# rchikhi/rust-seq2kminmers

Measured on AMD Instinct MI355X. Metric: input bases/s (Gbp/s) for k-min-mer extraction, l=31 k=10 d=0.01, higher is better.
Workload: dtype u32

## Files before the change

### rust-seq2kminmers_amd/csrc/s2k_api.hip

```cpp
#include "../../include/s2k.h"
#include "s2k_dev.h"
#include "s2k_hostcopy.h"

#include <math.h>
#include <stdio.h>
#include <stdlib.h>
#include <string.h>
#include <string>
#include <algorithm>
#include <atomic>
#include <chrono>
#include <condition_variable>
#include <thread>
#include <memory>
#include <mutex>
#include <sys/mman.h>
#include <vector>

using namespace s2k;

static_assert(offsetof(Counts, path) == offsetof(s2k_counts, path), "Counts must start with s2k_counts");

namespace {

// ... 116 lines not shown
    bool pinned[9] = {};
    explicit HostOwner(std::shared_ptr<HostPool> hp) : pool(std::move(hp)) {}
    template <typename T> T *take(int slot, uint64_t n) {
        p[slot] = pool->get((size_t)n * sizeof(T), &cap[slot], &pinned[slot]);
        return (T *)p[slot];
    }
    ~HostOwner() {
        for (int i = 0; i < 9; i++) pool->put(p[i], cap[i], pinned[i]);
    }
};

struct DevBuf {
    void *p = nullptr;
    size_t bytes = 0;
    hipError_t ensure(size_t need) {
        if (need <= bytes) return hipSuccess;
        if (p) {
            hipError_t e = hipFree(p);
            p = nullptr;
            bytes = 0;
            if (e != hipSuccess) return e;
        }
        size_t want = need + need / 8 + 4096;
        hipError_t e = hipMalloc(&p, want);
        if (e != hipSuccess) return e;
        bytes = want;
        return hipSuccess;
    }
    void release() {
        if (p) (void)hipFree(p);
        p = nullptr;
        bytes = 0;
    }
};

constexpr uint32_t MAX_DESC_CHUNKS = 64;
constexpr size_t CTRL_XOR_OFF = (sizeof(Counts) + 255) & ~(size_t)255;
constexpr size_t CTRL_CURSORS_OFF = CTRL_XOR_OFF + XOR_SHARDS * sizeof(uint64_t);

struct Arena {
    char *base;
    size_t off, cap;
    template <class T> T *take(size_t n) {
        size_t o = (off + 255) & ~(size_t)255;
        off = o + n * sizeof(T);
        return base ? reinterpret_cast<T *>(base + o) : nullptr;
    }
};

struct Call {
    const uint8_t *d_bases = nullptr;
    const uint64_t *d_read_off = nullptr;
    uint64_t n_reads = 0, n_bases = 0;
    s2k_params params{};
    s2k_device_out out{};
    Sem sem{};
    uint32_t bound = 0;
    bool serial = false;
    bool desc_run = false;
    bool full_runs = false;
    bool legacy = false;
    uint64_t pool_cap = 0;
    uint64_t slab_cap = 0;
    bool valid = false;
};

}

struct s2k_ctx {
    int device = 0;
    hipStream_t stream = nullptr;
    bool user_stream = false;
    bool has_pipes = false;
    hipStream_t p = nullptr;
    hipEvent_t done_ev = nullptr;
    bool done_valid = false;
    hipEvent_t entry_ev = nullptr;
    DevBuf ws, in_bases, in_off, outbuf, realign;
    DevBuf in_bases2, in_off2, outbuf2;
    DevBuf count_tab;
    hipStream_t s_in = nullptr, s_out = nullptr;
    std::vector<hipEvent_t> chunk_ev;
    uint32_t rec_per_tile_hint = 0;
    s2k_ctx *chain_prev = nullptr;
    hipEvent_t tiles_done = nullptr;
    bool tiles_done_valid = false;
    uint32_t desc_chunks = 0;
    uint32_t lookback_giveups = 0;
    bool force_full_runs = false;
    bool trace = false;
    bool poison_ws = false;
    uint8_t poison_byte = 0;
    uint64_t host_batch = 1ull << 29;
    Counts *d_counts = nullptr;
    Counts *h_counts = nullptr;
    uint64_t *d_xor = nullptr;
    uint64_t *d_cursors = nullptr;
    std::vector<hipEvent_t> evs;
    size_t ev_used = 0;
    hipEvent_t *ev = nullptr;
    bool timing = false, timed = false;
    Call call;
    bool pending = false;
    s2k_status pending_status = S2K_OK;
    std::string err;
    s2k::HostStager stager;
    s2k::HostStager stager_out;
    std::shared_ptr<HostPool> host_pool = std::make_shared<HostPool>();
};

namespace {
std::mutex g_ctx_mu;
std::vector<s2k_ctx *> g_live_ctx;

struct PipePair {
    hipStream_t p = nullptr, k = nullptr;
    int refs = 0;
};
std::vector<PipePair> g_pipes;
}

namespace {
hipError_t ensure_pipes(s2k_ctx *ctx) {
    if (ctx->has_pipes) return hipSuccess;
    hipError_t e = hipSetDevice(ctx->device);
    if (e != hipSuccess) return e;
    std::lock_guard<std::mutex> lk(g_ctx_mu);
    if (g_pipes.size() <= (size_t)ctx->device) g_pipes.resize((size_t)ctx->device + 1);
    PipePair &pp = g_pipes[ctx->device];
    if (!pp.p) {
        hipStream_t p = nullptr, spacer = nullptr, k = nullptr;
        e = hipStreamCreateWithFlags(&p, hipStreamNonBlocking);
        if (e == hipSuccess) e = hipStreamCreateWithFlags(&spacer, hipStreamNonBlocking);
        if (e == hipSuccess) e = hipStreamCreateWithFlags(&k, hipStreamNonBlocking);
        if (spacer) (void)hipStreamDestroy(spacer);
        if (e != hipSuccess) {
            if (p) (void)hipStreamDestroy(p);
            if (k) (void)hipStreamDestroy(k);
            return e;
        }
        pp.p = p;
        pp.k = k;
    }
    pp.refs++;
    ctx->has_pipes = true;
    ctx->p = pp.p;
    if (!ctx->user_stream) ctx->stream = pp.k;
    return hipSuccess;
}

hipError_t mark_done(s2k_ctx *ctx) {
    hipError_t e = hipEventRecord(ctx->done_ev, ctx->stream);
    if (e == hipSuccess) ctx->done_valid = true;
    return e;
}
}

namespace s2k {
HostStager &ctx_stager(s2k_ctx *c) { return c->stager; }
hipStream_t ctx_stream(s2k_ctx *c) {
    (void)ensure_pipes(c);
    return c->stream;
}
hipError_t ctx_mark(s2k_ctx *c) { return mark_done(c); }
hipError_t ctx_sync(s2k_ctx *c) {
    hipError_t e = mark_done(c);
// ... 182 lines not shown
        rec.ovf_cursor = (unsigned long long *)pool_cursor;
        if (pass == 0) {
            S2K_TRY(ctx->ws.ensure(a.off + 256), "workspace allocation");
            a.base = (char *)ctx->ws.p;
        }
    }
    if (c.serial) {
        tile_cnt = mn_cnt;
        tile_goff = mn_off;
        tile_rec_off = mn_off;
    }

    const bool tm = ctx->timing;
    ctx->timed = tm;
    S2K_TRY(ensure_pipes(ctx), "stream create");
    hipStream_t const sp = ctx->p, sk = ctx->stream;
    while (ctx->chunk_ev.size() < (size_t)n_chunks) {
        hipEvent_t e;
        S2K_TRY(hipEventCreateWithFlags(&e, hipEventDisableTiming), "event create");
        ctx->chunk_ev.push_back(e);
    }
    if (!ctx->tiles_done) S2K_TRY(hipEventCreateWithFlags(&ctx->tiles_done, hipEventDisableTiming), "event create");
    if (tm) {
        if (ctx->evs.size() < (ctx->ev_used + 1) * 6) {
            for (int i = 0; i < 6; i++) {
                hipEvent_t e;
                S2K_TRY(hipEventCreate(&e), "event create");
                ctx->evs.push_back(e);
            }
        }
        ctx->ev = &ctx->evs[ctx->ev_used * 6];
        ctx->ev_used++;
    }
    if (ctx->user_stream) {
        S2K_TRY(hipEventRecord(ctx->entry_ev, sk), "event");
        S2K_TRY(hipStreamWaitEvent(sp, ctx->entry_ev, 0), "stream wait (entry)");
    } else if (ctx->done_valid && hipEventQuery(ctx->done_ev) != hipSuccess) {
        S2K_TRY(hipStreamWaitEvent(sp, ctx->done_ev, 0), "stream wait (previous call)");
    }
    if (tm) S2K_TRY(hipEventRecord(ctx->ev[0], sp), "event");
    S2K_TRY(hipMemsetAsync(ctx->d_counts, 0, CTRL_CURSORS_OFF + (size_t)CURSOR_WORDS * (use_desc ? n_chunks : 1) * sizeof(uint64_t), sp),
            "memset counters, xor shards, cursors");
    auto hand_over = [&]() -> s2k_status {
        S2K_TRY(hipEventRecord(ctx->tiles_done, sp), "event");
        ctx->tiles_done_valid = true;
        if (tm) S2K_TRY(hipEventRecord(ctx->ev[2], sp), "event");
        S2K_TRY(hipEventRecord(ctx->chunk_ev[0], sp), "event");
        S2K_TRY(hipStreamWaitEvent(sk, ctx->chunk_ev[0], 0), "stream wait");
        return S2K_OK;
    };
    if (c.serial) {
        S2K_TRY(launch_validate_read_off(c.d_read_off, n_reads, n_bases, &ctx->d_counts->bad_input, sp), "read table validation");
        if (tm) S2K_TRY(hipEventRecord(ctx->ev[1], sp), "event");
        S2K_TRY(launch_serial_count(c.d_bases, c.d_read_off, n_reads, n_bases, c.sem, mn_cnt, sp), "serial count kernel");
        S2K_TRY(launch_scan_u32(mn_cnt, n_reads, mn_off, scan_tmp, 0, sp), "scan");
        S2K_TRY(launch_serial_write(c.d_bases, c.d_read_off, n_reads, n_bases, c.sem, mn_off, rec, ctx->d_counts, sp), "serial write kernel");
        s2k_status hs = hand_over();
        if (hs != S2K_OK) return hs;
    } else {
        if (!use_desc) S2K_TRY(hipMemsetAsync(mn_cnt, 0, (n_reads + 1) * sizeof(uint32_t), sp), "memset mn_cnt");
        S2K_TRY(launch_read_table(c.d_read_off, n_reads, n_bases, n_tiles, &ctx->d_counts->bad_input, tile_read0,
                                  use_desc ? (unsigned long long *)d_agg : nullptr, agg_pack(0, 0, 0, 0, true, true), sp),
                "read table kernel");
        Sem sem = c.sem;
        sem.read_runs = nullptr;
        sem.tile_heads = nullptr;
        if (want_runs) {
            if (c.full_runs) {
                S2K_TRY(launch_read_run_counts(c.d_bases, c.d_read_off, n_reads, n_bases, run_blk, run_off, run_tmp, read_runs, nullptr, sp),
                        "run count kernels");
                sem.read_runs = read_runs;
            } else {
                S2K_TRY(hipMemsetAsync(tile_heads, 0, n_tiles * sizeof(uint32_t), sp), "memset tile head words");
                sem.tile_heads = tile_heads;
            }
        }
        const uint32_t tile_mode = tile_mode_of(sem);
        if (use_desc) {
            Desc dz{};
            dz.agg = d_agg;
            dz.meta = d_meta;
            dz.state = d_state;
            dz.k = c.sem.k;
            dz.spec_n = ctx->rec_per_tile_hint ? ctx->rec_per_tile_hint : 192u;
            dz.km_capacity = o.km_capacity;
            dz.mn_capacity = o.mn_capacity;
            dz.o_km_off = (unsigned long long *)o.km_off;
            dz.o_hash = (unsigned long long *)o.hash;
            dz.o_start = o.start;
            dz.o_end = o.end;
            dz.o_rev = o.rev;
            dz.o_mn_off = (unsigned long long *)mn_off;
            dz.o_mn_j = o.mn_j;
            dz.o_mn_jend = o.mn_jend;
            dz.o_mn_hash = o.mn_hash;
            dz.xor_shards = (unsigned long long *)ctx->d_xor;
            if (tm) S2K_TRY(hipEventRecord(ctx->ev[1], sp), "event");
            if (tm && n_chunks > 1) S2K_TRY(hipEventRecord(ctx->ev[3], sk), "event");
            for (uint32_t ch = 0; ch < n_chunks; ch++) {
                auto cut = [&](uint32_t i) -> uint64_t {
                    static const double tail = getenv("S2K_DESC_TAIL") ? atof(getenv("S2K_DESC_TAIL")) : 0.0;
                    if (i >= n_chunks) return n_tiles;
                    if (tail <= 0.0 || tail >= 1.0 || n_chunks < 2) return n_tiles * i / n_chunks;
                    return (uint64_t)((double)n_tiles * (1.0 - tail) * (double)i / (double)(n_chunks - 1));
                };
                const uint64_t T0 = cut(ch), T1 = cut(ch + 1);
                const bool last = ch + 1 == n_chunks;
                S2K_TRY(launch_tile_minimizers(c.d_bases, c.d_read_off, n_reads, n_bases, T1, tile_read0, sem, tile_mode, rec,
                                               pool_cursor + (size_t)CURSOR_WORDS * ch, nullptr, nullptr, nullptr, ctx->d_counts, &dz, T0, sp),
                        "tiled minimizer kernel");
                if (last) {
                    S2K_TRY(hipEventRecord(ctx->tiles_done, sp), "event");
                    ctx->tiles_done_valid = true;
                    if (tm) S2K_TRY(hipEventRecord(ctx->ev[2], sp), "event");
                }
                S2K_TRY(hipEventRecord(ctx->chunk_ev[ch], sp), "event");
                S2K_TRY(hipStreamWaitEvent(sk, ctx->chunk_ev[ch], 0), "stream wait");
                if (tm && n_chunks == 1) S2K_TRY(hipEventRecord(ctx->ev[3], sk), "event");
#ifdef S2K_DEBUG_KNOBS
                static const bool nokm = getenv("S2K_DEBUG_NOKM") != nullptr;
                if (nokm) continue;
#endif
                S2K_TRY(launch_desc_scan(T0, T1, dz, d_scan, ctx->d_counts, sk), "tile word scan");
                S2K_TRY(launch_desc_kminmers(T0, T1, n_tiles, n_reads, dz, rec, ctx->d_counts, sk, last && !(chained && c.sem.hpc)), "k-min-mer kernel");
            }
            if (tm) S2K_TRY(hipEventRecord(ctx->ev[4], sk), "event");
            S2K_TRY(launch_finalize(ctx->d_counts, ctx->d_xor, (const uint64_t *)&d_state[n_tiles].gmn, (const uint64_t *)&d_state[n_tiles].g,
                                    o.km_capacity, o.mn_capacity, sk),
                    "finalize kernel");
            S2K_TRY(hipMemcpyAsync(ctx->h_counts, ctx->d_counts, sizeof(Counts), hipMemcpyDeviceToHost, sk), "counts copy");
            if (tm) S2K_TRY(hipEventRecord(ctx->ev[5], sk), "event");
            S2K_TRY(mark_done(ctx), "event");
            ctx->pending = true;
            return S2K_OK;
        }
        if (tm) S2K_TRY(hipEventRecord(ctx->ev[1], sp), "event");
        S2K_TRY(launch_tile_minimizers(c.d_bases, c.d_read_off, n_reads, n_bases, n_tiles, tile_read0, sem, tile_mode, rec, pool_cursor,
                                       tile_rec_off, tile_cnt, mn_cnt, ctx->d_counts, nullptr, 0, sp),
                "tiled minimizer kernel");
        s2k_status hs = hand_over();
        if (hs != S2K_OK) return hs;
        S2K_TRY(launch_scan_u32(tile_cnt, n_tiles, tile_goff, scan_tmp, 0, sk), "scan");
        S2K_TRY(launch_scan_u32(mn_cnt, n_reads, mn_off, scan_tmp, 0, sk), "scan");
    }
    S2K_TRY(launch_scan_u32(mn_cnt, n_reads, o.km_off, scan_tmp, c.sem.k, sk), "scan");
    if (tm) S2K_TRY(hipEventRecord(ctx->ev[3], sk), "event");
    S2K_TRY(launch_kminmers(n_tiles, tile_rec_off, tile_cnt, tile_goff, rec, mn_off, o.km_off, c.sem.k, o.km_capacity, o.hash,
                            o.start, o.end, o.rev, o.mn_capacity, o.mn_capacity ? o.mn_j : nullptr, o.mn_jend, o.mn_hash,
                            ctx->d_xor, ctx->d_counts, sk),
            "k-min-mer kernel");
    if (tm) S2K_TRY(hipEventRecord(ctx->ev[4], sk), "event");
    S2K_TRY(launch_finalize(ctx->d_counts, ctx->d_xor, mn_off + n_reads, o.km_off + n_reads, o.km_capacity, o.mn_capacity, sk),
            "finalize kernel");
    S2K_TRY(hipMemcpyAsync(ctx->h_counts, ctx->d_counts, sizeof(Counts), hipMemcpyDeviceToHost, sk), "counts copy");
    if (tm) S2K_TRY(hipEventRecord(ctx->ev[5], sk), "event");
    S2K_TRY(mark_done(ctx), "event");
    ctx->pending = true;
    return S2K_OK;
}

s2k_status finish(s2k_ctx *ctx, s2k_counts *counts) {
    if (!ctx->pending) {
        if (counts && ctx->call.valid) memcpy(counts, ctx->h_counts, sizeof(s2k_counts));
        return ctx->pending_status;
    }
    for (int attempt = 0; attempt < 4; attempt++) {
        S2K_TRY(hipEventSynchronize(ctx->done_ev), "event synchronize");
        ctx->pending = false;
        Counts *h = ctx->h_counts;
        Call &c = ctx->call;
        if (h->bad_input) {
            ctx->pending_status = (h->bad_input & ~(uint32_t)BAD_LONG) ? S2K_ERR_INVALID_ARG : S2K_ERR_READ_TOO_LONG;
            ctx->err = (h->bad_input & BAD_FIRST)   ? "d_read_off[0] != 0"
                       : (h->bad_input & BAD_ORDER) ? "d_read_off is not non-decreasing"
                       : (h->bad_input & BAD_END)   ? "d_read_off[n_reads] != n_bases"
                                                    : "a read is longer than 2^32-2 bases";
            c.valid = false;
            return ctx->pending_status;
        }
        if (h->need_legacy && c.desc_run) {
            c.legacy = true;
            if (ctx->trace) fprintf(stderr, "[s2k] re-run: the descriptor path met a tile it does not handle -> legacy path\n");
            s2k_status st = enqueue(ctx);
            if (st != S2K_OK) return st;
            continue;
        }
        if (h->need_runs && !c.full_runs) {
            c.full_runs = true;
            if (++ctx->lookback_giveups >= 2) ctx->force_full_runs = true;
            if (ctx->trace) fprintf(stderr, "[s2k] re-run: a look-back for run heads gave up -> runs of every read counted first\n");
            s2k_status st = enqueue(ctx);
            if (st != S2K_OK) return st;
            continue;
        }
        if (h->pool_overflow) {
            c.pool_cap = h->pool_needed + h->pool_needed / 64 + (uint64_t)TILE_BASES + 4096;
            if (ctx->trace) fprintf(stderr, "[s2k] re-run: record pool too small -> %llu records\n", (unsigned long long)c.pool_cap);
            s2k_status st = enqueue(ctx);
            if (st != S2K_OK) return st;
            continue;
        }
        if (c.desc_run && c.n_bases >= 64u * (uint64_t)TILE_BASES) {
            const double avg = (double)h->n_minimizers / ((double)c.n_bases / (double)TILE_BASES);
            const double want = avg + 2.5 * sqrt(avg + 1.0) + 3.0;
            ctx->rec_per_tile_hint = want >= 192.0 ? 192u : (uint32_t)want;
        }
        h->n_reads = c.n_reads;
        h->n_bases = c.n_bases;
        h->hash_bound = c.bound;
        h->path = c.serial ? 1u : (c.desc_run ? 0u : 2u);
        if (c.sem.dbg_skip & 32)
        {
            fprintf(stderr, "[s2k dbg] last wave finished %.1f us after the first; shader clock under the tiled kernel %.0f MHz (waves alive %.3f ms on average)\n",
                    (double)(h->dbg_cycles[0][0] - ~h->dbg_cycles[0][1]) * 0.01,
                    h->dbg_cycles[1][1] ? 100.0 * (double)h->dbg_cycles[1][0] / (double)h->dbg_cycles[1][1] : 0.0,
                    (double)h->dbg_cycles[1][1] * 1e-5 / (256.0 * 12.0));
#ifdef S2K_DEBUG_KNOBS
            if (const char *path = getenv("S2K_DEBUG_WAVE_DUMP")) {
                if (FILE *f = fopen(path, "w")) {
                    for (int i = 0; i < 4096; i++)
                        if (h->dbg_wave[i][0]) fprintf(f, "%d %llu %u %u\n", i, (unsigned long long)(h->dbg_wave[i][0] - ~h->dbg_cycles[0][1]), (unsigned)(h->dbg_wave[i][1] >> 32), (unsigned)h->dbg_wave[i][1]);
                    fclose(f);
                }
            }
#endif
        }
        if (c.sem.dbg_skip & 8) {
            fprintf(stderr, "[s2k dbg] phase cycles (sum over waves):");
            for (int i = 0; i < 16; i++) {
                unsigned long long sum = 0;
                for (int sh = 0; sh < 64; sh++) sum += h->dbg_cycles[sh][i];
                fprintf(stderr, " %llu", sum);
            }
            fprintf(stderr, "\n");
        }
        if (counts) memcpy(counts, h, sizeof(s2k_counts));
        ctx->pending_status = (h->km_overflow || h->mn_overflow) ? S2K_ERR_CAPACITY : S2K_OK;
        if (ctx->pending_status != S2K_OK) ctx->err = "device output capacity too small; see counts";
        return ctx->pending_status;
    }
    return fail(ctx, S2K_ERR_DEVICE, "workspace retry did not converge");
}

}

extern "C" {

int s2k_abi_version(void) { return S2K_ABI_VERSION; }

double s2k_density_for_bound(uint32_t bound) {
    if (bound == 0xFFFFFFFFu) return 1.0;
    const double d = ((double)bound + 0.5) / 4294967295.0;
    return hash_bound(d) == bound ? d : ((double)bound + 0.25) / 4294967295.0;
}

int s2k_device_count(void) {
    int n = 0;
    if (hipGetDeviceCount(&n) != hipSuccess) return 0;
    return n;
}

const char *s2k_strerror(s2k_status st) {
    switch (st) {
    case S2K_OK: return "ok";
    case S2K_ERR_INVALID_ARG: return "invalid argument";
    case S2K_ERR_L_RANGE: return "minimizer length l out of range";
    case S2K_ERR_K_RANGE: return "k-min-mer order k out of range";
    case S2K_ERR_READ_TOO_LONG: return "a read is longer than 2^32-2 bases";
    case S2K_ERR_DEVICE: return "HIP runtime error";
    case S2K_ERR_NOMEM: return "out of memory";
    case S2K_ERR_CAPACITY: return "device output capacity too small";
    case S2K_ERR_NO_DEVICE: return "no GPU visible (this library has no CPU path)";
    case S2K_ERR_NON_ASCII: return "reserved (not returned since ABI 2: every byte value is accepted)";
    }
    return "unknown status";
}

const char *s2k_last_error(const s2k_ctx *ctx) { return ctx ? ctx->err.c_str() : "no context"; }

uint32_t s2k_hash_bound(double density) { return hash_bound(density); }

s2k_ctx *s2k_create(int device, s2k_status *status) {
    s2k_status dummy;
    if (!status) status = &dummy;
    int n = 0;
    if (hipGetDeviceCount(&n) != hipSuccess || n <= 0) {
        *status = S2K_ERR_NO_DEVICE;
        return nullptr;
    }
    if (device < 0 || device >= n) {
        *status = S2K_ERR_INVALID_ARG;
        return nullptr;
    }
    if (hipSetDevice(device) != hipSuccess) {
        *status = S2K_ERR_DEVICE;
        return nullptr;
    }
    s2k_ctx *ctx = new (std::nothrow) s2k_ctx();
    if (!ctx) {
        *status = S2K_ERR_NOMEM;
        return nullptr;
    }
    ctx->device = device;
    bool ok = hipEventCreateWithFlags(&ctx->done_ev, hipEventDisableTiming) == hipSuccess;
    ok = ok && hipEventCreateWithFlags(&ctx->entry_ev, hipEventDisableTiming) == hipSuccess;
    ok = ok && hipMalloc((void **)&ctx->d_counts, CTRL_CURSORS_OFF + (size_t)CURSOR_WORDS * MAX_DESC_CHUNKS * sizeof(uint64_t)) == hipSuccess;
    if (ok) {
        ctx->d_xor = reinterpret_cast<uint64_t *>(reinterpret_cast<char *>(ctx->d_counts) + CTRL_XOR_OFF);
        ctx->d_cursors = reinterpret_cast<uint64_t *>(reinterpret_cast<char *>(ctx->d_counts) + CTRL_CURSORS_OFF);
    }
    ok = ok && hipHostMalloc((void **)&ctx->h_counts, sizeof(Counts), hipHostMallocDefault) == hipSuccess;
    if (!ok) {
        *status = S2K_ERR_DEVICE;
        s2k_destroy(ctx);
        return nullptr;
    }
    memset(ctx->h_counts, 0, sizeof(Counts));
    if (const char *e = getenv("S2K_DESC_CHUNKS"))
        if (atoi(e) >= 1 && atoi(e) <= 64) ctx->desc_chunks = (uint32_t)atoi(e);
    if (const char *e = getenv("S2K_TRACE")) ctx->trace = atoi(e) != 0;
    if (const char *e = getenv("S2K_POISON_WS"))
        if (*e && atoi(e) >= 0 && atoi(e) <= 255) ctx->poison_ws = true, ctx->poison_byte = (uint8_t)atoi(e);
    if (const char *e = getenv("S2K_FULL_RUNS")) ctx->force_full_runs = atoi(e) != 0;
    {
        std::lock_guard<std::mutex> lk(g_ctx_mu);
        g_live_ctx.push_back(ctx);
    }
    *status = S2K_OK;
    return ctx;
}

void s2k_destroy(s2k_ctx *ctx) {
    if (!ctx) return;
    {
        std::lock_guard<std::mutex> lk(g_ctx_mu);
        for (size_t i = 0; i < g_live_ctx.size();) {
            if (g_live_ctx[i] == ctx) {
                g_live_ctx[i] = g_live_ctx.back();
                g_live_ctx.pop_back();
                continue;
            }
            if (g_live_ctx[i]->chain_prev == ctx) g_live_ctx[i]->chain_prev = nullptr;
            i++;
        }
    }
    (void)hipSetDevice(ctx->device);
    if (ctx->tiles_done_valid) (void)hipEventSynchronize(ctx->tiles_done);
    if (ctx->has_pipes) (void)s2k::ctx_sync(ctx);
    ctx->ws.release();
    ctx->in_bases.release();
    ctx->realign.release();
    ctx->in_off.release();
    ctx->outbuf.release();
    ctx->in_bases2.release();
    ctx->in_off2.release();
    ctx->outbuf2.release();
    ctx->count_tab.release();
    if (ctx->tiles_done) (void)hipEventDestroy(ctx->tiles_done);
    for (hipEvent_t e : ctx->chunk_ev) (void)hipEventDestroy(e);
    if (ctx->s_in) (void)hipStreamDestroy(ctx->s_in);
    if (ctx->s_out) (void)hipStreamDestroy(ctx->s_out);
    if (ctx->d_counts) (void)hipFree(ctx->d_counts);
    if (ctx->h_counts) (void)hipHostFree(ctx->h_counts);
    for (hipEvent_t e : ctx->evs) (void)hipEventDestroy(e);
    if (ctx->done_ev) (void)hipEventDestroy(ctx->done_ev);
    if (ctx->entry_ev) (void)hipEventDestroy(ctx->entry_ev);
    if (ctx->has_pipes) {
        std::lock_guard<std::mutex> lk(g_ctx_mu);
        PipePair &pp = g_pipes[ctx->device];
        if (--pp.refs == 0) {
            (void)hipStreamDestroy(pp.p);
            (void)hipStreamDestroy(pp.k);
            pp = PipePair();
        }
    }
    delete ctx;
}

s2k_status s2k_set_stream(s2k_ctx *ctx, void *hip_stream) {
    if (!ctx) return S2K_ERR_INVALID_ARG;
    if (ctx->pending) {
        s2k_status st = finish(ctx, nullptr);
        (void)st;
    }
    S2K_TRY(hipSetDevice(ctx->device), "set device");
    if (ctx->has_pipes) S2K_TRY(s2k::ctx_sync(ctx), "event synchronize");
    ctx->stream = (hipStream_t)hip_stream;
    ctx->user_stream = true;
    ctx->done_valid = false;
    return S2K_OK;
}

s2k_status s2k_chain_after(s2k_ctx *ctx, s2k_ctx *prev) {
    if (!ctx || prev == ctx) return S2K_ERR_INVALID_ARG;
    std::lock_guard<std::mutex> lk(g_ctx_mu);
    if (prev) {
        bool live = false;
        for (s2k_ctx *c : g_live_ctx) live = live || c == prev;
        if (!live || prev->device != ctx->device) return S2K_ERR_INVALID_ARG;
    }
    ctx->chain_prev = prev;
    return S2K_OK;
}

s2k_status s2k_enable_timing(s2k_ctx *ctx, int on) {
    if (!ctx) return S2K_ERR_INVALID_ARG;
// ... 557 lines not shown
```

### rust-seq2kminmers_amd/csrc/s2k_desc.hip

```cpp
#include "s2k_dev.h"
#include <cstdlib>
#include <type_traits>

namespace s2k {
namespace {

constexpr unsigned long long M48 = (1ull << 48) - 1ull;

struct PairState {
    uint64_t G, Gmn;
    uint32_t p;
};
__device__ inline PairState applied(PairState s, const AggF &a, uint32_t K1) {
    s.G += agg_windows(a, s.p, K1);
    s.Gmn += a.N;
    s.p = agg_p(a, s.p, K1);
    return s;
}
__device__ inline void st_agg(unsigned long long *w, const AggF &a) {
    w[0] = a.m_f;
    w[1] = a.C;
    w[2] = a.N;
    w[3] = (unsigned long long)a.q | ((unsigned long long)(a.dep ? 1 : 0) << 8) | ((unsigned long long)(a.pass ? 1 : 0) << 9);
}
// ... 27 lines not shown
        b.pass = (f & 512u) != 0;
        if (lane >= o) a = agg_then(b, a, K1);
    }
    return a;
}
__device__ inline bool scan_off(const Counts *counts) { return counts->need_legacy || counts->need_runs || counts->bad_input || counts->pool_overflow; }

template <bool PACKED>
__global__ __launch_bounds__(256) void desc_scan_reduce(const unsigned long long *__restrict__ in, uint64_t n, uint32_t K1,
                                                        unsigned long long *__restrict__ out, const Counts *__restrict__ counts) {
    const int lane = threadIdx.x & 63;
    const uint64_t c = (uint64_t)blockIdx.x * 4 + (threadIdx.x >> 6), i = c * 64 + lane;
    if (c * 64 >= n || scan_off(counts)) return;
    const AggF a = wave_scan_agg(i < n ? ld_level<PACKED>(in, i) : agg_identity(), lane, K1);
    if (lane == 63) st_agg(out + 4 * c, a);
}
__global__ __launch_bounds__(64) void desc_scan_top(const unsigned long long *__restrict__ in, uint64_t n, uint32_t K1,
                                                    unsigned long long *__restrict__ states, const TileState *__restrict__ init,
                                                    const Counts *__restrict__ counts) {
    const int lane = threadIdx.x;
    if (scan_off(counts)) return;
    PairState s{0, 0, 0};
    if (init) {
        s.G = init->g & M48;
        s.p = (uint32_t)(init->g >> 48) & 63u;
        s.Gmn = init->gmn;
    }
    for (uint64_t b0 = 0; b0 < n; b0 += 64) {
        const uint64_t i = b0 + lane;
        const AggF inc = wave_scan_agg(i < n ? ld_agg(in + 4 * i) : agg_identity(), lane, K1);
        AggF exc;
        exc.m_f = shfl_up64(inc.m_f, 1);
        exc.C = shfl_up64(inc.C, 1);
        exc.N = shfl_up64(inc.N, 1);
        const uint32_t f = (uint32_t)__shfl_up((int)(inc.q | (inc.dep ? 256u : 0u) | (inc.pass ? 512u : 0u)), 1);
        exc.q = f & 63u;
        exc.dep = (f & 256u) != 0;
        exc.pass = (f & 512u) != 0;
        if (lane == 0) exc = agg_identity();
        const PairState mine = applied(s, exc, K1);
        if (i < n) {
            states[3 * i] = mine.G;
            states[3 * i + 1] = mine.Gmn;
            states[3 * i + 2] = mine.p;
        }
        const PairState after = applied(s, inc, K1);
        s.G = ((uint64_t)(uint32_t)__shfl((int)(uint32_t)(after.G >> 32), 63) << 32) | (uint32_t)__shfl((int)(uint32_t)after.G, 63);
        s.Gmn = ((uint64_t)(uint32_t)__shfl((int)(uint32_t)(after.Gmn >> 32), 63) << 32) | (uint32_t)__shfl((int)(uint32_t)after.Gmn, 63);
        s.p = (uint32_t)__shfl((int)after.p, 63);
    }
}
template <bool PACKED>
__global__ __launch_bounds__(256) void desc_scan_expand(const unsigned long long *__restrict__ in, uint64_t n, uint32_t K1,
                                                        const unsigned long long *__restrict__ chunk_states, unsigned long long *__restrict__ out_states,
                                                        TileState *__restrict__ out_tiles, const Counts *__restrict__ counts) {
    const int lane = threadIdx.x & 63;
    const uint64_t c = (uint64_t)blockIdx.x * 4 + (threadIdx.x >> 6), i = c * 64 + lane;
    if (c * 64 >= n || scan_off(counts)) return;
    const PairState s0{chunk_states[3 * c], chunk_states[3 * c + 1], (uint32_t)chunk_states[3 * c + 2]};
    const AggF inc = wave_scan_agg(i < n ? ld_level<PACKED>(in, i) : agg_identity(), lane, K1);
    AggF exc;
    exc.m_f = shfl_up64(inc.m_f, 1);
    exc.C = shfl_up64(inc.C, 1);
    exc.N = shfl_up64(inc.N, 1);
    const uint32_t f = (uint32_t)__shfl_up((int)(inc.q | (inc.dep ? 256u : 0u) | (inc.pass ? 512u : 0u)), 1);
    exc.q = f & 63u;
    exc.dep = (f & 256u) != 0;
    exc.pass = (f & 512u) != 0;
    if (lane == 0) exc = agg_identity();
    const PairState mine = applied(s0, exc, K1);
    if (i < n) {
        if constexpr (PACKED) {
            out_tiles[i].g = ((unsigned long long)mine.p << 48) | mine.G;
            out_tiles[i].gmn = mine.Gmn;
            if (i + 1 == n) {
                const PairState tot = applied(s0, inc, K1);
                out_tiles[n].g = ((unsigned long long)tot.p << 48) | tot.G;
                out_tiles[n].gmn = tot.Gmn;
            }
        } else {
            out_states[3 * i] = mine.G;
            out_states[3 * i + 1] = mine.Gmn;
            out_states[3 * i + 2] = mine.p;
        }
    }
}

constexpr int DK_WAVES = 4;
constexpr int DK_KMAX = 32;

__device__ inline uint32_t dk_incl_scan(uint32_t v) {
    uint32_t t;
    t = (uint32_t)__builtin_amdgcn_update_dpp(0, (int)v, 0x111, 0xf, 0xf, false);
    uint32_t a = v + t;
    t = (uint32_t)__builtin_amdgcn_update_dpp(0, (int)v, 0x112, 0xf, 0xf, false);
    a += t;
    t = (uint32_t)__builtin_amdgcn_update_dpp(0, (int)v, 0x113, 0xf, 0xf, false);
    a += t;
    t = (uint32_t)__builtin_amdgcn_update_dpp(0, (int)a, 0x114, 0xf, 0xe, false);
    a += t;
    t = (uint32_t)__builtin_amdgcn_update_dpp(0, (int)a, 0x118, 0xf, 0xc, false);
    a += t;
    t = (uint32_t)__builtin_amdgcn_update_dpp(0, (int)a, 0x142, 0xa, 0xf, false);
    a += t;
    t = (uint32_t)__builtin_amdgcn_update_dpp(0, (int)a, 0x143, 0xc, 0xf, false);
    a += t;
    return a;
}
__device__ inline uint32_t dk_incl_xor(uint32_t v) {
    uint32_t t;
    t = (uint32_t)__builtin_amdgcn_update_dpp(0, (int)v, 0x111, 0xf, 0xf, false);
    uint32_t a = v ^ t;
    t = (uint32_t)__builtin_amdgcn_update_dpp(0, (int)v, 0x112, 0xf, 0xf, false);
    a ^= t;
    t = (uint32_t)__builtin_amdgcn_update_dpp(0, (int)v, 0x113, 0xf, 0xf, false);
    a ^= t;
    t = (uint32_t)__builtin_amdgcn_update_dpp(0, (int)a, 0x114, 0xf, 0xe, false);
    a ^= t;
    t = (uint32_t)__builtin_amdgcn_update_dpp(0, (int)a, 0x118, 0xf, 0xc, false);
    a ^= t;
    t = (uint32_t)__builtin_amdgcn_update_dpp(0, (int)a, 0x142, 0xa, 0xf, false);
    a ^= t;
    t = (uint32_t)__builtin_amdgcn_update_dpp(0, (int)a, 0x143, 0xc, 0xf, false);
    a ^= t;
    return a;
}
__device__ inline uint32_t dk_lane(uint32_t v, int src) { return (uint32_t)__builtin_amdgcn_readlane((int)v, src); }

constexpr int DK_STAGE_RECS = 192, DK_STAGE_BYTES = DK_STAGE_RECS * 20;
template <int KT, bool FULL, bool COAL = false>
__global__ __launch_bounds__(64 * DK_WAVES, 8) void desc_kminmer_kernel(uint64_t tile_begin, uint64_t tile_end, uint64_t n_tiles, uint64_t n_reads, Desc dz,
                                                                        Records rec, Counts *counts) {
    __shared__ unsigned long long s_ring[DK_WAVES][((KT > 0 && FULL) ? 32 : 64) + DK_KMAX];
    __shared__ uint4 s_seg[DK_WAVES][META_SEGS];
    __shared__ uint32_t s_jcar[DK_WAVES][DK_KMAX];
    const int lane = threadIdx.x & 63, w = __builtin_amdgcn_readfirstlane((int)(threadIdx.x >> 6));
    uint32_t *const s_cum_w = reinterpret_cast<uint32_t *>(&s_ring[w][DK_KMAX]);
    const uint64_t t = tile_begin + (uint64_t)blockIdx.x * DK_WAVES + w;
    if (t >= tile_end) return;
    const uint32_t off_flags = counts->need_legacy | counts->need_runs | counts->bad_input | counts->pool_overflow;
    const unsigned long long agw = t >= (uint64_t)lane ? dz.agg[t - lane] : 0ull;
    const TileState st = dz.state[t];
    const TileMeta *m = &dz.meta[t];
    const uint64_t base = m->rec_base, rs0 = m->rs0, t0 = t * (uint64_t)TILE_BASES;
    const uint32_t r0 = m->r0, nb = m->nb, nrd = m->nrd;
    const uint32_t segstart_raw = lane < META_SEGS ? m->segstart[lane] : 0u, rs16 = lane < META_SEGS ? m->rs16[lane] : 0u;
    const uint64_t slab = t * rec.slab_cap;
    uint32_t nh32 = rec.hash[slab + lane], npos = rec.j[slab + lane];
    constexpr bool KFIX = KT > 0;
    constexpr bool SERIAL = KFIX && FULL;
    uint32_t sp_h0 = 0, sp_h1 = 0, sp_h2 = 0, sp_p0 = 0, sp_p1 = 0, sp_p2 = 0;
    if constexpr (SERIAL) {
        if (3u * (uint32_t)lane < dz.spec_n) {
            const uint32_t *ph = rec.hash + slab + 3u * (uint32_t)lane, *pp = rec.j + slab + 3u * (uint32_t)lane;
            sp_h0 = ph[0], sp_h1 = ph[1], sp_h2 = ph[2];
            sp_p0 = pp[0], sp_p1 = pp[1], sp_p2 = pp[2];
        }
    }
    if (off_flags) return;
    const uint32_t k = KFIX ? (uint32_t)KT : dz.k, K1 = k - 1;
    const unsigned long long ag0 = ((unsigned long long)dk_lane((uint32_t)(agw >> 32), 0) << 32) | dk_lane((uint32_t)agw, 0);
    const AggF ag = agg_unpack(ag0);
    const uint32_t N = (uint32_t)ag.N;
    const uint64_t G = st.g & M48, Gmn = st.gmn;
    const uint32_t p_in = ag.dep ? (uint32_t)(st.g >> 48) & 63u : 0u;
    if (base != slab && (uint32_t)lane < N) {
// ... 329 lines not shown
#pragma unroll
            for (int mm = 0; mm < KT; mm++) {
                al[mm] = rot_lo(xl[mm], xh[mm], KT - 1 - mm);
                ah[mm] = rot_hi(xl[mm], xh[mm], KT - 1 - mm);
                bl[mm] = rot_lo(xl[mm], xh[mm], mm);
                bh[mm] = rot_hi(xl[mm], xh[mm], mm);
            }
            fl = al[0], fh = ah[0], rl = bl[0], rh = bh[0];
#pragma unroll
            for (int mm = 1; mm + 1 < KT; mm += 2) {
                fl = xor3(fl, al[mm], al[mm + 1]);
                fh = xor3(fh, ah[mm], ah[mm + 1]);
                rl = xor3(rl, bl[mm], bl[mm + 1]);
                rh = xor3(rh, bh[mm], bh[mm + 1]);
            }
            if constexpr (KT % 2 == 0) {
                fl ^= al[KT - 1];
                fh ^= ah[KT - 1];
                rl ^= bl[KT - 1];
                rh ^= bh[KT - 1];
            }
            rvv = ((uint64_t)rh << 32) | rl;
        } else {
            for (uint32_t mm = 0; mm < k; mm++) {
                const uint64_t xw = s_ring[w][lane + mm];
                const uint32_t xl = (uint32_t)xw, xh = (uint32_t)(xw >> 32);
                const uint32_t nfh = __builtin_amdgcn_alignbit(fh, fl, 31), nfl = __builtin_amdgcn_alignbit(fl, fh, 31);
                const uint32_t nrl = __builtin_amdgcn_alignbit(rh, rl, 1), nrh = __builtin_amdgcn_alignbit(rl, rh, 1);
                fl = nfl ^ xl;
                fh = nfh ^ xh;
                rl = nrl ^ xl;
                rh = nrh ^ xh;
            }
            rvv = rotl64(((uint64_t)rh << 32) | rl, K1);
        }
        const uint64_t f = ((uint64_t)fh << 32) | fl;
        const int src = ((lane - (int)K1) & 63) << 2;
        const uint32_t jsame = (uint32_t)__builtin_amdgcn_ds_bpermute(src, (int)j), jbefore = (uint32_t)__builtin_amdgcn_ds_bpermute(src, (int)jprev);
        const uint32_t jstart = (uint32_t)lane >= K1 ? jsame : jbefore;
        const uint64_t hmin = f < rvv ? f : rvv;
        if (win) {
            const uint32_t ot = i + sg.y;
            xacc ^= hmin;
            if (tile_fits) {
                t_hash[ot] = hmin;
                t_start[ot] = jstart;
                t_end[ot] = jend;
                t_rev[ot] = (uint8_t)(rvv < f);
            } else {
                const uint64_t o = G + (uint64_t)ot;
                if (o < dz.km_capacity) {
                    if (dz.o_hash) dz.o_hash[o] = hmin;
                    if (dz.o_start) dz.o_start[o] = jstart;
                    if (dz.o_end) dz.o_end[o] = jend;
                    if (dz.o_rev) dz.o_rev[o] = (uint8_t)(rvv < f);
                }
            }
        }
        if (!FULL && dz.mn_capacity && act) {
            const uint64_t g = Gmn + i;
            if (g < dz.mn_capacity) {
                dz.o_mn_j[g] = j;
                dz.o_mn_jend[g] = jend;
                dz.o_mn_hash[g] = h32;
            }
        }
        wave_sync();
        if ((uint32_t)lane >= 64u - K1) s_ring[w][lane - (64u - K1)] = xm;
        jprev = j;
    }
    }
    const uint32_t xl_all = dk_incl_xor((uint32_t)xacc), xh_all = dk_incl_xor((uint32_t)(xacc >> 32));
    if (lane == 63 && (xl_all | xh_all))
        atomicXor((unsigned long long *)&dz.xor_shards[t & (XOR_SHARDS - 1)], ((unsigned long long)xh_all << 32) | xl_all);
}

}

size_t desc_scan_tmp_words(uint64_t n_tiles) {
    const uint64_t n1 = (n_tiles + 63) / 64, n2 = (n1 + 63) / 64;
    return 7 * n1 + 7 * n2 + 16;
}

hipError_t launch_desc_scan(uint64_t tile_begin, uint64_t tile_end, Desc dz, unsigned long long *scan_tmp, const Counts *counts, hipStream_t st) {
    if (tile_end <= tile_begin) return hipSuccess;
    const uint64_t n = tile_end - tile_begin;
    const uint64_t n1 = (n + 63) / 64, n2 = (n1 + 63) / 64;
    unsigned long long *w1 = scan_tmp, *s1 = w1 + 4 * n1, *w2 = s1 + 3 * n1, *s2 = w2 + 4 * n2;
    const uint32_t K1 = dz.k - 1;
    const unsigned long long *agg = dz.agg + tile_begin;
    TileState *state = dz.state + tile_begin;
    hipLaunchKernelGGL(desc_scan_reduce<true>, dim3((unsigned)((n1 + 3) / 4)), dim3(256), 0, st, agg, n, K1, w1, counts);
    hipLaunchKernelGGL(desc_scan_reduce<false>, dim3((unsigned)((n2 + 3) / 4)), dim3(256), 0, st, w1, n1, K1, w2, counts);
    hipLaunchKernelGGL(desc_scan_top, dim3(1), dim3(64), 0, st, w2, n2, K1, s2, tile_begin ? (const TileState *)state : (const TileState *)nullptr, counts);
    hipLaunchKernelGGL(desc_scan_expand<false>, dim3((unsigned)((n2 + 3) / 4)), dim3(256), 0, st, w1, n1, K1, s2, s1, (TileState *)nullptr, counts);
    hipLaunchKernelGGL(desc_scan_expand<true>, dim3((unsigned)((n1 + 3) / 4)), dim3(256), 0, st, agg, n, K1, s1, (unsigned long long *)nullptr, state,
                       counts);
    return hipGetLastError();
}

hipError_t launch_desc_kminmers(uint64_t tile_begin, uint64_t tile_end, uint64_t n_tiles, uint64_t n_reads, Desc dz, Records rec, Counts *counts,
                                hipStream_t st, bool alone) {
    if (tile_end <= tile_begin) return hipSuccess;
    if (dz.k == 0 || dz.k > (uint32_t)DK_KMAX || rec.slab_cap < 64) return hipErrorInvalidValue;
    const dim3 g((unsigned)((tile_end - tile_begin + DK_WAVES - 1) / DK_WAVES)), b(64 * DK_WAVES);
    unsigned pad = 0;
#ifdef S2K_DEBUG_KNOBS
    if (const char *e = getenv("S2K_DEBUG_KM_LDS")) pad = (unsigned)atoi(e);
#endif
    const bool full = dz.o_hash && dz.o_start && dz.o_end && dz.o_rev && dz.mn_capacity == 0;
    static const bool no_coal = getenv("S2K_KM_NO_COAL") != nullptr;
    const bool coal = alone && full && !no_coal && (dz.k == 10 || dz.k == 5);
#define S2K_KM_GO(KT, F, C) \
    hipLaunchKernelGGL((desc_kminmer_kernel<KT, F, C>), g, b, (C) ? (unsigned)(DK_WAVES * DK_STAGE_BYTES) : pad, st, tile_begin, tile_end, n_tiles, n_reads, dz, rec, counts)
    switch (dz.k) {
    case 10: if (coal) S2K_KM_GO(10, true, true); else if (full) S2K_KM_GO(10, true, false); else S2K_KM_GO(10, false, false); break;
    case 5: if (coal) S2K_KM_GO(5, true, true); else if (full) S2K_KM_GO(5, true, false); else S2K_KM_GO(5, false, false); break;
    default: if (full) S2K_KM_GO(0, true, false); else S2K_KM_GO(0, false, false); break;
    }
#undef S2K_KM_GO
    return hipGetLastError();
}

}
```

### rust-seq2kminmers_amd/csrc/s2k_dev.h

```cpp
#pragma once
#include <hip/hip_runtime.h>
#include <stdint.h>

namespace s2k {

constexpr uint32_t SEED_A = 0x95c60474u, SEED_C = 0x62a02b4cu, SEED_G = 0x82572324u, SEED_T = 0x4be24456u;

__host__ __device__ inline uint32_t seed_h_scalar(uint32_t c) {
    return c == 'A' ? SEED_A : c == 'C' ? SEED_C : c == 'G' ? SEED_G : c == 'T' ? SEED_T : c == 'N' ? 0u : 1u;
}
__host__ __device__ inline uint32_t seed_rc_scalar(uint32_t c) {
    return c == 'A' ? SEED_T : c == 'C' ? SEED_G : c == 'G' ? SEED_C : c == 'T' ? SEED_A : c == 'N' ? 0u : 1u;
}
__host__ __device__ inline uint32_t seed_h_simd(uint32_t c) {
    uint32_t n = c & 15u;
    return n == 1 ? SEED_A : n == 3 ? SEED_C : n == 7 ? SEED_G : n == 4 ? SEED_T : 0u;
}
__host__ __device__ inline uint32_t seed_rc_simd(uint32_t c) {
    uint32_t n = c & 15u;
    return n == 1 ? SEED_T : n == 3 ? SEED_G : n == 7 ? SEED_C : n == 4 ? SEED_A : 0u;
}

#if defined(__HIP_DEVICE_COMPILE__)
__device__ __forceinline__ uint32_t xor3(uint32_t a, uint32_t b, uint32_t c) {
// ... 127 lines not shown
constexpr int META_SEGS = 32;
struct TileMeta {
    unsigned long long rec_base;
    unsigned long long rs0;
    uint32_t r0;
    uint16_t nb, nrd;
    uint16_t segstart[META_SEGS];
    uint16_t rs16[META_SEGS];
};
struct TileState {
    unsigned long long g;
    unsigned long long gmn;
};
constexpr uint32_t REC_SPAN_MAX = (1u << 18) - 1u;
struct Desc {
    unsigned long long *agg;
    TileMeta *meta;
    TileState *state;
    uint32_t k;
    uint32_t spec_n;
    unsigned long long km_capacity, mn_capacity;
    unsigned long long *o_km_off, *o_hash;
    uint32_t *o_start, *o_end;
    uint8_t *o_rev;
    unsigned long long *o_mn_off;
    uint32_t *o_mn_j, *o_mn_jend, *o_mn_hash;
    unsigned long long *xor_shards;
};

#define S2K_HIP_CHECK(expr)                                                      \
    do {                                                                         \
        hipError_t _e = (expr);                                                  \
        if (_e != hipSuccess) return _e;                                         \
    } while (0)

hipError_t launch_scan_u32(const uint32_t *in, uint64_t n, uint64_t *out , uint64_t *block_tmp,
                           uint32_t sub_k , hipStream_t st);
size_t scan_tmp_bytes(uint64_t n);

__host__ __device__ inline bool is_rle_char(uint32_t c) {
    const uint32_t d = (c & 0xDFu) - 'A';
    return d < 20u && ((0x82045u >> d) & 1u) != 0u;
}
__host__ __device__ inline bool run_head(uint32_t cur, uint32_t prev, bool rle) { return cur != prev || (rle && !is_rle_char(cur)); }

hipError_t launch_read_run_counts(const uint8_t *bases, const uint64_t *read_off, uint64_t n_reads, uint64_t n_bases,
                                  uint32_t *blk_cnt, uint64_t *blk_off, uint64_t *scan_tmp, uint32_t *runs, uint64_t *read_c0,
                                  hipStream_t st, bool rle = false);
hipError_t launch_hpc_segments(const uint8_t *bases, const uint64_t *read_off, uint64_t n_reads, uint64_t n_bases,
                               const uint64_t *hpc_off, const uint64_t *blk_off, const uint64_t *read_c0, uint32_t *seg_index, uint8_t *o_hpc,
                               uint32_t *o_pos, uint64_t capacity, hipStream_t st, bool rle = false);
size_t hpc_single_pass_words(uint64_t n_bases);
hipError_t launch_hpc_single_pass(const uint8_t *bases, const uint64_t *read_off, uint64_t n_reads, uint64_t n_bases, uint32_t *ws, uint64_t *o_hpc_off,
                                  uint8_t *o_hpc, uint32_t *o_pos, uint64_t capacity, uint32_t **fail_word, hipStream_t st, bool rle = false);
size_t hpc_segment_index_words(uint64_t n_bases);

hipError_t launch_validate_read_off(const uint64_t *read_off, uint64_t n_reads, uint64_t n_bases, uint32_t *bad, hipStream_t st);
hipError_t launch_read_table(const uint64_t *read_off, uint64_t n_reads, uint64_t n_bases, uint64_t n_tiles, uint32_t *bad, uint32_t *tile_read0,
                             unsigned long long *tile_words, unsigned long long word0, hipStream_t st);

hipError_t launch_synth(uint64_t seed, uint64_t first_base, uint64_t n, uint8_t *d, hipStream_t st);
hipError_t launch_fill_u64(unsigned long long *d, uint64_t n, unsigned long long v, hipStream_t st);
uint64_t synth_hifi_len(uint64_t seed, uint64_t r);
hipError_t launch_synth_hifi(uint64_t seed, uint64_t r0, uint64_t n_reads, const uint64_t *read_off, uint8_t *d, hipStream_t st);

hipError_t launch_serial_count(const uint8_t *bases, const uint64_t *read_off, uint64_t n_reads, uint64_t n_bases, Sem sem,
                               uint32_t *mn_cnt, hipStream_t st);
hipError_t launch_serial_write(const uint8_t *bases, const uint64_t *read_off, uint64_t n_reads, uint64_t n_bases, Sem sem,
                               const uint64_t *mn_off, Records rec, Counts *counts, hipStream_t st);

hipError_t launch_kminmers(uint64_t n_tiles, const uint64_t *tile_rec_off, const uint32_t *tile_cnt,
                           const uint64_t *tile_goff, Records rec, const uint64_t *mn_off, const uint64_t *km_off,
                           uint32_t k, uint64_t km_capacity, uint64_t *o_hash, uint32_t *o_start, uint32_t *o_end,
                           uint8_t *o_rev, uint64_t mn_capacity, uint32_t *o_mn_j, uint32_t *o_mn_jend,
                           uint32_t *o_mn_hash, uint64_t *xor_shards, const Counts *counts, hipStream_t st);
hipError_t launch_finalize(Counts *counts, const uint64_t *xor_shards, const uint64_t *mn_total, const uint64_t *km_total,
                           uint64_t km_capacity, uint64_t mn_capacity, hipStream_t st);

hipError_t launch_tile_minimizers(const uint8_t *bases, const uint64_t *read_off, uint64_t n_reads, uint64_t n_bases,
                                  uint64_t n_tiles, const uint32_t *tile_read0, Sem sem, uint32_t mode, Records rec,
                                  uint64_t *pool_cursor, uint64_t *tile_rec_off, uint32_t *tile_cnt, uint32_t *mn_cnt,
                                  Counts *counts, const Desc *desc, uint64_t tile_begin, hipStream_t st);
hipError_t launch_desc_scan(uint64_t tile_begin, uint64_t tile_end, Desc dz, unsigned long long *scan_tmp ,
                            const Counts *counts, hipStream_t st);
size_t desc_scan_tmp_words(uint64_t n_tiles);
hipError_t launch_desc_kminmers(uint64_t tile_begin, uint64_t tile_end, uint64_t n_tiles, uint64_t n_reads, Desc dz, Records rec, Counts *counts,
                                hipStream_t st, bool alone);

hipError_t launch_hpc_count(const uint8_t *bases, const uint64_t *read_off, uint64_t n_reads, uint32_t *run_cnt, hipStream_t st,
                            bool rle = false);
hipError_t launch_hpc_write(const uint8_t *bases, const uint64_t *read_off, uint64_t n_reads, const uint64_t *hpc_off,
                            uint8_t *o_hpc, uint32_t *o_pos, uint64_t capacity, hipStream_t st, bool rle = false);

enum { FX_TOT_RECORDS = 0, FX_TOT_BASES, FX_TOT_ERR, FX_TOT_BLANK, FX_TOT_LASTLINE, FX_TOT_NEWLINES, FX_N_TOTALS };
size_t fx_ws_bytes(uint64_t n);
bool fx_malformed(const uint64_t *h_totals, uint64_t n, int fastq);
hipError_t fx_parse_count(const uint8_t *d_raw, uint64_t n, int fastq, void *ws, uint64_t *d_totals, hipStream_t st);
hipError_t fx_parse_write(const uint8_t *d_raw, uint64_t n, int fastq, void *ws, uint64_t *d_totals, uint8_t *d_bases,
                          uint64_t bases_cap, uint64_t *d_read_off, uint64_t off_cap, hipStream_t st);

}
```

Baseline: 1842.

## Replace five-launch tile-word scan with two-launch reduce/expand scan

```diff
diff --git a/rust-seq2kminmers_amd/csrc/s2k_api.hip b/rust-seq2kminmers_amd/csrc/s2k_api.hip
--- a/rust-seq2kminmers_amd/csrc/s2k_api.hip
+++ b/rust-seq2kminmers_amd/csrc/s2k_api.hip
@@ -222,6 +222,12 @@
     hipStream_t s_in = nullptr, s_out = nullptr;
     std::vector<hipEvent_t> chunk_ev;
     uint32_t rec_per_tile_hint = 0;
+    struct {
+        int32_t mode = -1;
+        uint32_t l = 0, k = 0;
+        double density = 0.0;
+    } hint_key;
+    bool scan_five = false;
     s2k_ctx *chain_prev = nullptr;
     hipEvent_t tiles_done = nullptr;
     bool tiles_done_valid = false;
@@ -570,6 +576,8 @@
             dz.meta = d_meta;
             dz.state = d_state;
             dz.k = c.sem.k;
+            if (ctx->hint_key.mode != c.params.mode || ctx->hint_key.l != c.params.l || ctx->hint_key.k != c.params.k || ctx->hint_key.density != c.params.density)
+                ctx->rec_per_tile_hint = 0;
             dz.spec_n = ctx->rec_per_tile_hint ? ctx->rec_per_tile_hint : 192u;
             dz.km_capacity = o.km_capacity;
             dz.mn_capacity = o.mn_capacity;
@@ -609,7 +617,7 @@
                 static const bool nokm = getenv("S2K_DEBUG_NOKM") != nullptr;
                 if (nokm) continue;
 #endif
-                S2K_TRY(launch_desc_scan(T0, T1, dz, d_scan, ctx->d_counts, sk), "tile word scan");
+                S2K_TRY(launch_desc_scan(T0, T1, dz, d_scan, ctx->d_counts, sk, ctx->scan_five), "tile word scan");
                 S2K_TRY(launch_desc_kminmers(T0, T1, n_tiles, n_reads, dz, rec, ctx->d_counts, sk, last && !(chained && c.sem.hpc)), "k-min-mer kernel");
             }
             if (tm) S2K_TRY(hipEventRecord(ctx->ev[4], sk), "event");
@@ -692,6 +700,7 @@
             const double avg = (double)h->n_minimizers / ((double)c.n_bases / (double)TILE_BASES);
             const double want = avg + 2.5 * sqrt(avg + 1.0) + 3.0;
             ctx->rec_per_tile_hint = want >= 192.0 ? 192u : (uint32_t)want;
+            ctx->hint_key.mode = c.params.mode, ctx->hint_key.l = c.params.l, ctx->hint_key.k = c.params.k, ctx->hint_key.density = c.params.density;
         }
         h->n_reads = c.n_reads;
         h->n_bases = c.n_bases;
@@ -810,6 +819,7 @@
     if (const char *e = getenv("S2K_POISON_WS"))
         if (*e && atoi(e) >= 0 && atoi(e) <= 255) ctx->poison_ws = true, ctx->poison_byte = (uint8_t)atoi(e);
     if (const char *e = getenv("S2K_FULL_RUNS")) ctx->force_full_runs = atoi(e) != 0;
+    if (const char *e = getenv("S2K_SCAN_FIVE")) ctx->scan_five = atoi(e) != 0;
     {
         std::lock_guard<std::mutex> lk(g_ctx_mu);
         g_live_ctx.push_back(ctx);
diff --git a/rust-seq2kminmers_amd/csrc/s2k_desc.hip b/rust-seq2kminmers_amd/csrc/s2k_desc.hip
--- a/rust-seq2kminmers_amd/csrc/s2k_desc.hip
+++ b/rust-seq2kminmers_amd/csrc/s2k_desc.hip
@@ -133,6 +133,90 @@
             out_states[3 * i] = mine.G;
             out_states[3 * i + 1] = mine.Gmn;
             out_states[3 * i + 2] = mine.p;
+        }
+    }
+}
+
+constexpr int DS2_THREADS = 256, DS2_PER_LANE = 16, DS2_TILES = DS2_THREADS * DS2_PER_LANE;
+constexpr uint64_t DS2_MAX_BLOCKS = 512;
+
+__device__ inline AggF agg_of_lane(const AggF &a, int src) {
+    AggF b;
+    b.m_f = ((uint64_t)(uint32_t)__shfl((int)(uint32_t)(a.m_f >> 32), src) << 32) | (uint32_t)__shfl((int)(uint32_t)a.m_f, src);
+    b.C = ((uint64_t)(uint32_t)__shfl((int)(uint32_t)(a.C >> 32), src) << 32) | (uint32_t)__shfl((int)(uint32_t)a.C, src);
+    b.N = ((uint64_t)(uint32_t)__shfl((int)(uint32_t)(a.N >> 32), src) << 32) | (uint32_t)__shfl((int)(uint32_t)a.N, src);
+    const uint32_t f = (uint32_t)__shfl((int)(a.q | (a.dep ? 256u : 0u) | (a.pass ? 512u : 0u)), src);
+    b.q = f & 63u;
+    b.dep = (f & 256u) != 0;
+    b.pass = (f & 512u) != 0;
+    return b;
+}
+__device__ inline AggF ds2_lane_fold(const unsigned long long *__restrict__ in, uint64_t i0, uint64_t n, uint32_t K1, unsigned long long (&wd)[DS2_PER_LANE]) {
+    const unsigned long long idw = agg_pack(0, 0, 0, 0, true, true);
+#pragma unroll
+    for (int r = 0; r < DS2_PER_LANE; r++) wd[r] = i0 + r < n ? in[i0 + r] : idw;
+    AggF a = agg_unpack(wd[0]);
+#pragma unroll
+    for (int r = 1; r < DS2_PER_LANE; r++) a = agg_then(a, agg_unpack(wd[r]), K1);
+    return a;
+}
+__global__ __launch_bounds__(DS2_THREADS) void desc_scan2_reduce(const unsigned long long *__restrict__ in, uint64_t n, uint32_t K1,
+                                                                 unsigned long long *__restrict__ out) {
+    __shared__ unsigned long long s_w[DS2_THREADS / 64][4];
+    const int lane = threadIdx.x & 63, w = threadIdx.x >> 6;
+    unsigned long long wd[DS2_PER_LANE];
+    const AggF inc = wave_scan_agg(ds2_lane_fold(in, (uint64_t)blockIdx.x * DS2_TILES + (uint64_t)threadIdx.x * DS2_PER_LANE, n, K1, wd), lane, K1);
+    if (lane == 63) st_agg(s_w[w], inc);
+    __syncthreads();
+    if (threadIdx.x == 0) {
+        AggF x = ld_agg(s_w[0]);
+        for (int v = 1; v < DS2_THREADS / 64; v++) x = agg_then(x, ld_agg(s_w[v]), K1);
+        st_agg(out + 4 * (uint64_t)blockIdx.x, x);
+    }
+}
+__global__ __launch_bounds__(DS2_THREADS, 4) void desc_scan2_expand(const unsigned long long *__restrict__ in, uint64_t n, uint32_t K1,
+                                                                 const unsigned long long *__restrict__ words, TileState *out_tiles,
+                                                                 const TileState *init) {
+    __shared__ unsigned long long s_w[DS2_THREADS / 64][4];
+    __shared__ unsigned long long s_s0[3];
+    const int lane = threadIdx.x & 63, w = threadIdx.x >> 6;
+    const uint64_t i0 = (uint64_t)blockIdx.x * DS2_TILES + (uint64_t)threadIdx.x * DS2_PER_LANE;
+    unsigned long long wd[DS2_PER_LANE];
+    const AggF inc = wave_scan_agg(ds2_lane_fold(in, i0, n, K1, wd), lane, K1);
+    if (lane == 63) st_agg(s_w[w], inc);
+    if (w == 0) {
+        PairState s{0, 0, 0};
+        if (init) {
+            s.G = init->g & M48;
+            s.p = (uint32_t)(init->g >> 48) & 63u;
+            s.Gmn = init->gmn;
+        }
+        for (uint64_t b0 = 0; b0 < (uint64_t)blockIdx.x; b0 += 64) {
+            const uint64_t i = b0 + lane;
+            const AggF x = wave_scan_agg(i < (uint64_t)blockIdx.x ? ld_agg(words + 4 * i) : agg_identity(), lane, K1);
+            s = applied(s, agg_of_lane(x, 63), K1);
+        }
+        if (lane == 0) s_s0[0] = s.G, s_s0[1] = s.Gmn, s_s0[2] = s.p;
+    }
+    __syncthreads();
+    PairState s{s_s0[0], s_s0[1], (uint32_t)s_s0[2]};
+    for (int v = 0; v < w; v++) s = applied(s, ld_agg(s_w[v]), K1);
+    AggF exc = agg_of_lane(inc, (lane + 63) & 63);
+    if (lane == 0) exc = agg_identity();
+    s = applied(s, exc, K1);
+#pragma unroll
+    for (int r = 0; r < DS2_PER_LANE; r++) {
+        const uint64_t i = i0 + r;
+        if (i < n && !(init && i == 0)) {
+            out_tiles[i].g = ((unsigned long long)s.p << 48) | s.G;
+            out_tiles[i].gmn = s.Gmn;
+        }
+        unsigned long long wr = wd[r];
+        asm volatile("" : "+v"(wr));
+        s = applied(s, agg_unpack(wr), K1);
+        if (i + 1 == n) {
+            out_tiles[n].g = ((unsigned long long)s.p << 48) | s.G;
+            out_tiles[n].gmn = s.Gmn;
         }
     }
 }
@@ -628,7 +712,8 @@
     return 7 * n1 + 7 * n2 + 16;
 }
 
-hipError_t launch_desc_scan(uint64_t tile_begin, uint64_t tile_end, Desc dz, unsigned long long *scan_tmp, const Counts *counts, hipStream_t st) {
+hipError_t launch_desc_scan(uint64_t tile_begin, uint64_t tile_end, Desc dz, unsigned long long *scan_tmp, const Counts *counts, hipStream_t st,
+                            bool five_launches) {
     if (tile_end <= tile_begin) return hipSuccess;
     const uint64_t n = tile_end - tile_begin;
     const uint64_t n1 = (n + 63) / 64, n2 = (n1 + 63) / 64;
@@ -636,6 +721,13 @@
     const uint32_t K1 = dz.k - 1;
     const unsigned long long *agg = dz.agg + tile_begin;
     TileState *state = dz.state + tile_begin;
+    static_assert(DS2_TILES == 64 * 64, "one block of the two-launch scan per word of the second level: its words fit where those are kept");
+    if (!five_launches && n2 <= DS2_MAX_BLOCKS) {
+        hipLaunchKernelGGL(desc_scan2_reduce, dim3((unsigned)n2), dim3(DS2_THREADS), 0, st, agg, n, K1, scan_tmp);
+        hipLaunchKernelGGL(desc_scan2_expand, dim3((unsigned)n2), dim3(DS2_THREADS), 0, st, agg, n, K1, (const unsigned long long *)scan_tmp, state,
+                           tile_begin ? (const TileState *)state : (const TileState *)nullptr);
+        return hipGetLastError();
+    }
     hipLaunchKernelGGL(desc_scan_reduce<true>, dim3((unsigned)((n1 + 3) / 4)), dim3(256), 0, st, agg, n, K1, w1, counts);
     hipLaunchKernelGGL(desc_scan_reduce<false>, dim3((unsigned)((n2 + 3) / 4)), dim3(256), 0, st, w1, n1, K1, w2, counts);
     hipLaunchKernelGGL(desc_scan_top, dim3(1), dim3(64), 0, st, w2, n2, K1, s2, tile_begin ? (const TileState *)state : (const TileState *)nullptr, counts);
diff --git a/rust-seq2kminmers_amd/csrc/s2k_dev.h b/rust-seq2kminmers_amd/csrc/s2k_dev.h
--- a/rust-seq2kminmers_amd/csrc/s2k_dev.h
+++ b/rust-seq2kminmers_amd/csrc/s2k_dev.h
@@ -233,7 +233,7 @@
                                   uint64_t *pool_cursor, uint64_t *tile_rec_off, uint32_t *tile_cnt, uint32_t *mn_cnt,
                                   Counts *counts, const Desc *desc, uint64_t tile_begin, hipStream_t st);
 hipError_t launch_desc_scan(uint64_t tile_begin, uint64_t tile_end, Desc dz, unsigned long long *scan_tmp ,
-                            const Counts *counts, hipStream_t st);
+                            const Counts *counts, hipStream_t st, bool five_launches = false);
 size_t desc_scan_tmp_words(uint64_t n_tiles);
 hipError_t launch_desc_kminmers(uint64_t tile_begin, uint64_t tile_end, uint64_t n_tiles, uint64_t n_reads, Desc dz, Records rec, Counts *counts,
                                 hipStream_t st, bool alone);
```

Result: no change. 1843 (median of 6 runs) (+0.1%).
